# iiscleap/NeuralPlda

Hardware: AMD Instinct MI355X
Metric: scored trial-pairs/sec (512-d xvec) (higher is better)
Workload: dtype f32; 1 GPU; cfg1: 1048576 trial pairs/GPU/step, 512->150->150 NPLDA, scoring only (fused NeuralPlda.forward, inputs resident in HBM); xvector_dim=512, layer1_LDA_dim=150, layer2_PLDA_spkfactor_dim=150, params=kaldi-init truncated to 150, parallelism=trial-list shard x1, backend=single process, ranks_in_group=1

## Files before the change

neuralplda_amd/csrc/nplda_fwd_dispatch.h:

```cpp
#pragma once
#include <cstdlib>
#include "nplda_fwd_kernel.h"
#include "nplda_fwd_small.h"
#include "nplda_fwd_v2.h"
#include "nplda_fwd_v3.h"
#include "nplda_fwd_v5.h"
#include "nplda_fwd_v6.h"
#include "nplda_fwd_mid.h"

namespace nplda {

template <int MODE>
static inline int launch_fwd_v2(FwdArgs a, const NpldaLayout& L, hipStream_t st) {
    constexpr int WAVES = 8;
    const long long per_block = (MODE == MODE_EMBED ? 32 : 16) * WAVES;
    const long long blocks = (a.n + per_block - 1) / per_block;
    if (blocks > 0x7fffffffLL) return NPLDA_EINVAL;
    dim3 grid((unsigned)blocks), block(WAVES * 64);
#define NPLDA_LAUNCH(NBV) \
    hipLaunchKernelGGL((nplda_fwd_v2_kernel<NBV, MODE, WAVES, false, (NBV == 2 ? 4 : 2)>), grid, block, 0, st, a)
    switch (L.NB) {
        case 2: NPLDA_LAUNCH(2); break;
        case 4: NPLDA_LAUNCH(4); break;
        case 8: NPLDA_LAUNCH(8); break;
        case 10: NPLDA_LAUNCH(10); break;
        case 11: NPLDA_LAUNCH(11); break;
        case 12: NPLDA_LAUNCH(12); break;
        default: return NPLDA_EUNSUPPORTED;
    }
#undef NPLDA_LAUNCH
    return nplda_launch_status();
}

template <int MODE, int XM = 0>
static inline int launch_fwd_v3(FwdArgs a, const NpldaLayout& L, hipStream_t st) {
    constexpr int WAVES = 8;
    const long long per_block = (MODE == MODE_EMBED ? 32 : 16) * WAVES;
    const long long ntiles = (a.n + per_block - 1) / per_block;
    if (ntiles > 0x7fffffffLL) return NPLDA_EINVAL;
    int dev = 0, cus = 0;
    if (hipGetDevice(&dev) != hipSuccess ||
        hipDeviceGetAttribute(&cus, hipDeviceAttributeMultiprocessorCount, dev) != hipSuccess || cus <= 0)
        cus = 256;
    const long long blocks = ntiles < cus ? ntiles : cus;
    dim3 grid((unsigned)blocks), block(WAVES * 64);
#define NPLDA_LAUNCH(NBV) \
    hipLaunchKernelGGL((nplda_fwd_v3_kernel<NBV, MODE, WAVES, XM, (NBV == 2 ? 4 : 2)>), grid, block, 0, st, a, (int)ntiles)
    switch (L.NB) {
        case 2: NPLDA_LAUNCH(2); break;
        case 4: NPLDA_LAUNCH(4); break;
        case 8: NPLDA_LAUNCH(8); break;
        case 10: NPLDA_LAUNCH(10); break;
        default: return NPLDA_EUNSUPPORTED;
    }
#undef NPLDA_LAUNCH
    return nplda_launch_status();
}

template <int XM = 0>
static inline int launch_fwd_v5(FwdArgs a, const NpldaLayout& L, hipStream_t st) {
    constexpr int WAVES = 8;
    const long long ntiles = (a.n + 16 * WAVES - 1) / (16 * WAVES);
    if (ntiles > 0x7fffffffLL) return NPLDA_EINVAL;
    int dev = 0, cus = 0;
    if (hipGetDevice(&dev) != hipSuccess ||
        hipDeviceGetAttribute(&cus, hipDeviceAttributeMultiprocessorCount, dev) != hipSuccess || cus <= 0)
        cus = 256;
    const long long blocks = ntiles < cus ? ntiles : cus;
    dim3 grid((unsigned)blocks), block(WAVES * 64);
    switch (L.NB) {
        case 11: hipLaunchKernelGGL((nplda_fwd_v5_kernel<11, WAVES, 2, 6, 1, XM>), grid, block, 0, st, a, (int)ntiles); break;
        case 12: hipLaunchKernelGGL((nplda_fwd_v5_kernel<12, WAVES, 4, 4, 1, XM>), grid, block, 0, st, a, (int)ntiles); break;
        default: return NPLDA_EUNSUPPORTED;
    }
    return nplda_launch_status();
}

static inline bool fwd_v6_ok(const NpldaLayout& L) { return L.NB == 10 && L.D1 == 150 && L.D2 == 150; }
template <int XM = 0>
static inline int launch_fwd_v6(FwdArgs a, const NpldaLayout& L, hipStream_t st) {
    constexpr int WAVES = 8;
    const long long ntiles = (a.n + 16 * WAVES - 1) / (16 * WAVES);
    if (ntiles > 0x7fffffffLL) return NPLDA_EINVAL;
    if (!fwd_v6_ok(L)) return NPLDA_EUNSUPPORTED;
    int dev = 0, cus = 0;
    if (hipGetDevice(&dev) != hipSuccess ||
        hipDeviceGetAttribute(&cus, hipDeviceAttributeMultiprocessorCount, dev) != hipSuccess || cus <= 0)
        cus = 256;
    const long long blocks = ntiles < cus ? ntiles : cus;
    hipLaunchKernelGGL((nplda_fwd_v6_kernel<10, 6, WAVES, 2, 5, 3, XM>), dim3((unsigned)blocks), dim3(WAVES * 64), 0, st, a, (int)ntiles);
    return nplda_launch_status();
}
template <int XM = 0>
static inline int launch_fwd_stream(FwdArgs a, const NpldaLayout& L, hipStream_t st) {
    static const bool no_v6 = getenv("NPLDA_FWD_NO_V6") != nullptr && getenv("NPLDA_FWD_NO_V6")[0] == '1';
    if (fwd_v6_ok(L) && !no_v6) return launch_fwd_v6<XM>(a, L, st);
    if (L.NB <= 10) return launch_fwd_v3<MODE_PAIR, XM>(a, L, st);
    return launch_fwd_v5<XM>(a, L, st);
}

template <int MODE>
static inline int launch_fwd_small(FwdArgs a, const NpldaLayout& L, hipStream_t st) {
    const long long per_block = (MODE == MODE_EMBED ? 32 : 16);
    const long long blocks = (a.n + per_block - 1) / per_block;
    dim3 grid((unsigned)blocks), block(256);
#define NPLDA_LAUNCH(NBV) hipLaunchKernelGGL((nplda_fwd_small_kernel<NBV, MODE>), grid, block, 0, st, a)
#define NPLDA_LAUNCH32(NBV)                                                                           \
    if (L.KS1 == 32 && L.D0 == 512) hipLaunchKernelGGL((nplda_fwd_small_kernel<NBV, MODE, 32>), grid, block, 0, st, a); \
    else NPLDA_LAUNCH(NBV)
    switch (L.NB) {
        case 2: NPLDA_LAUNCH(2); break;
        case 4: NPLDA_LAUNCH(4); break;
        case 8: NPLDA_LAUNCH(8); break;
        case 10: NPLDA_LAUNCH32(10); break;
        case 11: NPLDA_LAUNCH32(11); break;
        case 12: NPLDA_LAUNCH(12); break;
        default: return NPLDA_EUNSUPPORTED;
    }
#undef NPLDA_LAUNCH32
#undef NPLDA_LAUNCH
    return nplda_launch_status();
}

static inline int mid_cus() {
    int dev = 0, cus = 0;
    if (hipGetDevice(&dev) != hipSuccess ||
        hipDeviceGetAttribute(&cus, hipDeviceAttributeMultiprocessorCount, dev) != hipSuccess || cus <= 0)
        cus = 256;
    return cus;
}
template <bool EMBED = false>
static inline int launch_fwd_mid(FwdArgs a, const NpldaLayout& L, hipStream_t st) {
    const long long nh = EMBED ? (a.n + 15) / 16 : (a.n + 7) / 8;
    const int cus = mid_cus();
    long long grid = nh <= cus ? nh : ((nh + 1) / 2 < cus ? (nh + 1) / 2 : cus);
    if (grid < 1) grid = 1;
    const long long c = (nh + grid - 1) / grid;
    const long long r = nh - grid * (c - 1);
    if (c > 0x7fffffffLL) return NPLDA_EINVAL;
    const bool half = !(r == grid && (c & 1) == 0);
    const bool idx = a.ia != nullptr;
#define NPLDA_LAUNCH(NBV, HV, IV) \
    hipLaunchKernelGGL((nplda_fwd_mid_kernel<NBV, EMBED, HV, IV>), dim3((unsigned)grid), dim3(256), 0, st, a, (int)c, (int)r)
#define NPLDA_LAUNCH_H(NBV, HV) do { if (idx) { NPLDA_LAUNCH(NBV, HV, true); } else { NPLDA_LAUNCH(NBV, HV, false); } } while (0)
    switch (L.NB) {
        case 10: if (half) NPLDA_LAUNCH_H(10, true); else NPLDA_LAUNCH_H(10, false); break;
        case 11: if (half) NPLDA_LAUNCH_H(11, true); else NPLDA_LAUNCH_H(11, false); break;
        default: return NPLDA_EUNSUPPORTED;
    }
#undef NPLDA_LAUNCH_H
#undef NPLDA_LAUNCH
    return nplda_launch_status();
}

template <int MODE>
static inline int launch_fwd_old(FwdArgs a, const NpldaLayout& L, hipStream_t st) {
    a.D0 = L.D0; a.KS1 = L.KS1;
    a.oW2 = L.oW2; a.ob1 = L.ob1; a.ob2 = L.ob2; a.oQ = L.oQ; a.oP = L.oP; a.total = L.total;
    const long long units = (MODE == MODE_EMBED ? (a.n + 1) / 2 : a.n);
    if (units <= 256 * 64) return launch_fwd_small<MODE>(a, L, st);
    if constexpr (MODE == MODE_PAIR) return launch_fwd_stream<0>(a, L, st);
    return launch_fwd_v2<MODE>(a, L, st);
}

enum { FWD_SMALL = 0, FWD_MID = 1, FWD_STREAM = 2, FWD_SPLIT = 3 };
static inline long long pair_split_point(long long n, int cus) { return (n / 128 / cus) * 128 * cus; }
static inline int pair_kernel_choice(long long n, const NpldaLayout& L, int cus, long long* cost = nullptr, bool allow_split = true) {
    long long dummy;
    if (!cost) cost = &dummy;
    static const bool no_mid = getenv("NPLDA_FWD_NO_MID") != nullptr && getenv("NPLDA_FWD_NO_MID")[0] == '1';
    const bool mid_ok = !no_mid && (L.NB == 10 || L.NB == 11) && L.D0 == 512 && L.KS1 == 32;
    static const long long small_max = getenv("NPLDA_FWD_SMALL_MAX") ? atoll(getenv("NPLDA_FWD_SMALL_MAX")) : -1;
    const long long round_cost = L.NB == 10 ? 1000 : 1150;
    *cost = 120;
    if (mid_ok && small_max < 0 && n <= 8LL * cus) return FWD_MID;
    *cost = 190;
    if (n <= (small_max >= 0 ? small_max : 16LL * cus)) return FWD_SMALL;
    const long long rounds = ((n + 127) / 128 + cus - 1) / cus;
    const long long t_stream = 50 + rounds * round_cost;
    *cost = n <= 64LL * cus ? 190 * ((n + 16LL * cus - 1) / (16LL * cus)) : t_stream;
    if (!mid_ok) return n <= 64LL * cus ? FWD_SMALL : FWD_STREAM;
    const long long ch = ((n + 7) / 8 + cus - 1) / cus;
    const long long t_mid = 40 + (ch / 2) * (L.NB == 10 ? 133 : 168) + (ch & 1) * (L.NB == 10 ? 93 : 118);
    int best = t_mid < t_stream ? FWD_MID : FWD_STREAM;
    *cost = t_mid < t_stream ? t_mid : t_stream;
    static const bool no_split = getenv("NPLDA_FWD_NO_SPLIT") != nullptr && getenv("NPLDA_FWD_NO_SPLIT")[0] == '1';
    const long long full = pair_split_point(n, cus);
    if (allow_split && !no_split && full > 0 && full < n) {
        long long t_rem = 0;
        pair_kernel_choice(n - full, L, cus, &t_rem, false);
        const long long t_split = 50 + (full / 128 / cus) * round_cost + t_rem;
        if (t_split + 30 < *cost) {
            *cost = t_split;
            best = FWD_SPLIT;
        }
    }
    return best;
}

template <int MODE>
static inline int launch_fwd(FwdArgs a, const NpldaLayout& L, hipStream_t st) {
    if constexpr (MODE == MODE_PAIR) {
        const int cus = mid_cus();
        const int k = pair_kernel_choice(a.n, L, cus);
        a.D0 = L.D0; a.KS1 = L.KS1;
        a.oW2 = L.oW2; a.ob1 = L.ob1; a.ob2 = L.ob2; a.oQ = L.oQ; a.oP = L.oP; a.total = L.total;
        if (k == FWD_MID) return launch_fwd_mid<false>(a, L, st);
        if (k == FWD_SMALL) return launch_fwd_small<MODE>(a, L, st);
        if (k == FWD_SPLIT && a.ia == nullptr && a.ib == nullptr) {
            const long long full = pair_split_point(a.n, cus);
            FwdArgs b = a;
            b.xa += full * a.ldx; b.xb += full * a.ldx; b.out_s += full; b.n = a.n - full;
            a.n = full;
            if (int rc = launch_fwd_stream<0>(a, L, st)) return rc;
            const int kr = pair_kernel_choice(b.n, L, cus, nullptr, false);
            if (kr == FWD_MID) return launch_fwd_mid<false>(b, L, st);
            if (kr == FWD_SMALL) return launch_fwd_small<MODE>(b, L, st);
            return launch_fwd_stream<0>(b, L, st);
        }
        return launch_fwd_stream<0>(a, L, st);
    }
    if constexpr (MODE == MODE_EMBED) {
        if (a.out_y == nullptr && pair_kernel_choice((a.n + 1) / 2, L, mid_cus(), nullptr, false) == FWD_MID) {
            a.D0 = L.D0; a.KS1 = L.KS1;
            a.oW2 = L.oW2; a.ob1 = L.ob1; a.ob2 = L.ob2; a.oQ = L.oQ; a.oP = L.oP; a.total = L.total;
            return launch_fwd_mid<true>(a, L, st);
        }
    }
    return launch_fwd_old<MODE>(a, L, st);
}

static inline int launch_fwd_pairs_bf16rows(FwdArgs a, const NpldaLayout& L, hipStream_t st) {
    const int k = pair_kernel_choice(a.n, L, mid_cus());
    if (k != FWD_STREAM && k != FWD_SPLIT) return NPLDA_EUNSUPPORTED;
    a.D0 = L.D0; a.KS1 = L.KS1;
    a.oW2 = L.oW2; a.ob1 = L.ob1; a.ob2 = L.ob2; a.oQ = L.oQ; a.oP = L.oP; a.total = L.total;
    return launch_fwd_stream<2>(a, L, st);
}

static inline const char* pair_kernel_name(long long n, const NpldaLayout& L) {
    switch (pair_kernel_choice(n, L, mid_cus())) {
        case FWD_SPLIT:
            return pair_kernel_name(pair_split_point(n, mid_cus()), L);
        case FWD_SMALL: return "nplda_fwd_small_kernel (4 waves share a 16-pair tile, feature-split)";
        case FWD_MID: return "nplda_fwd_mid_kernel (balanced 16-pair tiles, K-split layer 1, groups of 2 tiles)";
        default:
            if (fwd_v6_ok(L) && !(getenv("NPLDA_FWD_NO_V6") != nullptr && getenv("NPLDA_FWD_NO_V6")[0] == '1'))
                return "nplda_fwd_v6_kernel (persistent, 9 feature blocks on 16x16x4 MFMAs + 6 features on 4x4x1 MFMAs)";
            return L.NB <= 10 ? "nplda_fwd_v3_kernel (persistent, 8 waves x 16 pairs, weights through LDS)"
                              : "nplda_fwd_v5_kernel (persistent, LDS-DMA weight chunks, layer 2 by output groups)";
    }
}

static inline int check_model(int D0, int D1, int D2) {
    if (D0 <= 0 || D1 <= 0 || D2 <= 0 || (D0 % 4) != 0) return NPLDA_EINVAL;
    if (!nplda_dims_ok(D0, D1, D2)) return NPLDA_EUNSUPPORTED;
    return NPLDA_OK;
}

static inline bool rows_ok(const float* x, int64_t ld, int D) {
    return x && ld >= D && (ld % 4) == 0 && nplda_aligned16(x);
}

}
```

neuralplda_amd/csrc/nplda_fwd_v6.h:

```cpp
#pragma once
#include "nplda_fwd_kernel.h"

namespace nplda {

template <int NB, int TF, int WAVES, int KPB = 2, int G1 = 5, int G2 = 3, int XM = 0, int ABL = 0, int NCH = 2>
__global__ __launch_bounds__(WAVES * 64, WAVES / 4) void nplda_fwd_v6_kernel(const FwdArgs a, int ntiles) {
    constexpr int NM = NB - 1;
    constexpr int NQ = (TF + 3) / 4;
    constexpr int STEP4 = NB * 64;
    constexpr int CH1 = STEP4 * KPB;
    constexpr int NSEG1 = CH1 / 64;
    constexpr int NGR = (NM + G1 - 1) / G1;
    constexpr int NG = (NM + G2 - 1) / G2;
    constexpr int NSEG2 = NB * (G2 + 1);
    constexpr int CH2 = NSEG2 * 64;
    constexpr int CH = CH1 > CH2 ? CH1 : CH2;
    static_assert(TF >= 1 && TF <= 16 && NM >= 1 && NQ <= NGR && NQ <= NG, "tail quads ride with the MFMA groups");
    __shared__ f32x4 wbuf[2][CH];
    __shared__ f32x4 cvec[4][NB * 4];
    __shared__ f32x4 sink[64];

    const int tid = threadIdx.x;
    const int lane = tid & 63;
    const int wave = __builtin_amdgcn_readfirstlane(tid >> 6);
    const int j = lane & 15;
    const int g = lane >> 4;
    const int tl = 16 * g + (j & 3);

    const f32x4* Wall = reinterpret_cast<const f32x4*>(a.packed);
    const long long w2base4 = (long long)(a.oW2 / 4);
    for (int i = tid; i < 4 * NB * 4; i += WAVES * 64) {
        const int v = i / (NB * 4), e = i % (NB * 4);
        const size_t o = v == 0 ? a.ob1 : (v == 1 ? a.ob2 : (v == 2 ? a.oQ : a.oP));
        cvec[v][e] = reinterpret_cast<const f32x4*>(a.packed + o)[e];
    }
    const f32x4* b1p = cvec[0];
    const f32x4* b2p = cvec[1];
    const f32x4* Qp = cvec[2];
    const f32x4* Pp = cvec[3];
    const int KS1 = a.KS1;
    const int D0 = a.D0;
    const int NC1 = (KS1 + KPB - 1) / KPB;

    auto seg_dma = [&](const f32x4* src, f32x4* dst) {
        unsigned lo = (unsigned)lane * 16u;
        asm volatile("" : "+v"(lo));
        __builtin_amdgcn_global_load_lds((const __attribute__((address_space(1))) void*)(reinterpret_cast<const char*>(src) + lo),
                                         (__attribute__((address_space(3))) void*)dst, 16, 0, 0);
    };
    auto dma_l1 = [&](int c, f32x4* dst) {
        const f32x4* src = Wall + (long long)c * CH1;
#pragma unroll
        for (int i = 0; i < (NSEG1 + WAVES - 1) / WAVES; ++i) {
            const int sgm = wave + WAVES * i;
            const bool live = sgm < NSEG1;
            seg_dma(src + (live ? sgm : 0) * 64, live ? dst + sgm * 64 : sink);
        }
    };
    auto dma_l2 = [&](int nb0, int gc, f32x4* dst) {
        const int per = gc + 1;
        const int nseg = NB * per;
#pragma unroll
        for (int i = 0; i < (NSEG2 + WAVES - 1) / WAVES; ++i) {
            const int sgm = wave + WAVES * i;
            const bool live = sgm < nseg;
            const int sg = live ? sgm : 0;
            const int kb = sg / per, u = sg - kb * per;
            const int blk = u < gc ? nb0 + u : NM;
            seg_dma(Wall + w2base4 + (long long)kb * STEP4 + blk * 64, live ? dst + sgm * 64 : sink);
        }
    };
    auto chunk_fence = [&]() {
        __builtin_amdgcn_s_waitcnt(0x0070);
        __builtin_amdgcn_s_barrier();
        __builtin_amdgcn_sched_barrier(0);
    };
    auto kgroups_sum = [&](float v) {
        v = wave_xor_add(v, 16);
        return wave_xor_add(v, 32);
    };
    auto as_block = [&](const float (&u)[TF]) {
        f32x4 blk = {0.f, 0.f, 0.f, 0.f};
#pragma unroll
        for (int r = 0; r < 4; ++r) {
#pragma unroll
            for (int gg = 0; gg < 4; ++gg)
                if (4 * gg + r < TF) blk[r] = (g == gg) ? u[4 * gg + r] : blk[r];
        }
        return blk;
    };

    auto tile_rows = [&](long long t, long long& t0, long long& r) {
        t0 = (t * WAVES + wave) * 16;
        r = t0 + j;
    };
    long long tile = blockIdx.x;
    long long t0, row;
    tile_rows(tile, t0, row);
    bool ok = row < a.n;
    if (!ok) row = a.n - 1;
    const float* sa = x_row<XM>(a.xa, row, a.ldx);
    const float* sb = x_row<XM>(a.xb, row, a.ldx);

    dma_l1(0, wbuf[0]);
    f32x4 xa[KPB], xb[KPB];
#pragma unroll
    for (int s = 0; s < KPB; ++s) {
        xa[s] = load_xrow<XM>(sa, 16 * s + 4 * g, D0);
        xb[s] = load_xrow<XM>(sb, 16 * s + 4 * g, D0);
    }
    __syncthreads();
    chunk_fence();
    int par = 0;

    for (;;) {
        const long long tile_n = tile + gridDim.x;
        long long t0_n, row_n;
        tile_rows(tile_n, t0_n, row_n);
        const bool ok_n = row_n < a.n;
        if (!ok_n) row_n = a.n - 1;
        const float* sa_n = x_row<XM>(a.xa, row_n, a.ldx);
        const float* sb_n = x_row<XM>(a.xb, row_n, a.ldx);

        f32x4 accA[NB], accB[NB];
#pragma unroll
        for (int nb = 0; nb < NM; ++nb) {
            accA[nb] = b1p[4 * nb + g];
            accB[nb] = accA[nb];
        }
        f32x4 qA[NQ][NCH], qB[NQ][NCH];
#pragma unroll
        for (int q = 0; q < NQ; ++q) {
#pragma unroll
            for (int h = 0; h < NCH; ++h) {
                qA[q][h] = f32x4{0.f, 0.f, 0.f, 0.f};
                qB[q][h] = qA[q][h];
            }
        }

        auto chunk = [&](int c, f32x4 (&xc)[KPB], f32x4 (&yc)[KPB], f32x4 (&xn)[KPB], f32x4 (&yn)[KPB]) {
            const bool more = (c + 1 < NC1);
            f32x4* nxt = wbuf[par ^ 1];
            if (more) dma_l1(c + 1, nxt);
            else dma_l2(0, (G2 < NM ? G2 : NM), nxt);
#pragma unroll
            for (int s = 0; s < KPB; ++s) {
                const int ks = more ? KPB * (c + 1) + s : KPB * c + s;
                xn[s] = load_xrow<XM>(sa, 16 * ks + 4 * g, D0);
                yn[s] = load_xrow<XM>(sb, 16 * ks + 4 * g, D0);
            }
            const f32x4* w = wbuf[par];
#pragma unroll
            for (int s = 0; s < KPB; ++s) {
                if (KPB * c + s < KS1) {
#pragma unroll
                    for (int gr = 0; gr < NGR; ++gr) {
                        const int nb0 = gr * G1;
                        f32x4 av[G1];
#pragma unroll
                        for (int u = 0; u < G1; ++u)
                            if (nb0 + u < NM) av[u] = w[s * STEP4 + (nb0 + u) * 64 + lane];
#pragma unroll
                        for (int r = 0; r < 4; ++r) {
#pragma unroll
                            for (int u = 0; u < G1; ++u) {
                                if (nb0 + u < NM) {
                                    accA[nb0 + u] = __builtin_amdgcn_mfma_f32_16x16x4f32(av[u][r], xc[s][r], accA[nb0 + u], 0, 0, 0);
                                    accB[nb0 + u] = __builtin_amdgcn_mfma_f32_16x16x4f32(av[u][r], yc[s][r], accB[nb0 + u], 0, 0, 0);
                                }
                            }
                        }
                        if (gr < NQ && ABL != 1) {
                            const f32x4 wq = w[s * STEP4 + NM * 64 + tl + 4 * gr];
#pragma unroll
                            for (int r = 0; r < 4; ++r) {
                                qA[gr][r % NCH] = __builtin_amdgcn_mfma_f32_4x4x1f32(wq[r], xc[s][r], qA[gr][r % NCH], 0, 0, 0);
                                qB[gr][r % NCH] = __builtin_amdgcn_mfma_f32_4x4x1f32(wq[r], yc[s][r], qB[gr][r % NCH], 0, 0, 0);
                            }
                        }
                    }
                }
            }
            chunk_fence();
            par ^= 1;
        };
        f32x4 xan[KPB], xbn[KPB];
        int c = 0;
        for (; c + 1 < NC1; c += 2) {
            chunk(c, xa, xb, xan, xbn);
            chunk(c + 1, xan, xbn, xa, xb);
        }
        if (c < NC1) {
            chunk(c, xa, xb, xan, xbn);
#pragma unroll
            for (int s = 0; s < KPB; ++s) {
                xa[s] = xan[s];
                xb[s] = xbn[s];
            }
        }

        {
            float uA[TF], uB[TF];
#pragma unroll
            for (int f = 0; f < TF; ++f) {
                float sa_ = qA[f / 4][0][f % 4], sb_ = qB[f / 4][0][f % 4];
#pragma unroll
                for (int h = 1; h < NCH; ++h) {
                    sa_ += qA[f / 4][h][f % 4];
                    sb_ += qB[f / 4][h][f % 4];
                }
                uA[f] = kgroups_sum(sa_);
                uB[f] = kgroups_sum(sb_);
            }
            const f32x4 bt = b1p[4 * NM + g];
            accA[NM] = as_block(uA) + bt;
            accB[NM] = as_block(uB) + bt;
        }

        {
            float ssA = 0.f, ssB = 0.f;
#pragma unroll
            for (int nb = 0; nb < NB; ++nb) {
#pragma unroll
                for (int r = 0; r < 4; ++r) {
                    ssA = fmaf(accA[nb][r], accA[nb][r], ssA);
                    ssB = fmaf(accB[nb][r], accB[nb][r], ssB);
                }
            }
            ssA = wave_xor_add(ssA, 16); ssA = wave_xor_add(ssA, 32);
            ssB = wave_xor_add(ssB, 16); ssB = wave_xor_add(ssB, 32);
            const float invA = 1.0f / fmaxf(sqrtf(ssA), 1e-12f);
            const float invB = 1.0f / fmaxf(sqrtf(ssB), 1e-12f);
#pragma unroll
            for (int nb = 0; nb < NB; ++nb) {
                accA[nb] *= invA;
                accB[nb] *= invB;
            }
        }

        float part = 0.f;
#pragma unroll
        for (int gi = 0; gi < NG; ++gi) {
            const int nb0 = gi * G2;
            const int gc = (NM - nb0) < G2 ? (NM - nb0) : G2;
            const int per = gc + 1;
            f32x4 zA[G2], zB[G2];
#pragma unroll
            for (int u = 0; u < G2; ++u) {
                if (u < gc) {
                    zA[u] = b2p[4 * (nb0 + u) + g];
                    zB[u] = zA[u];
                }
            }
            f32x4 zqA[2] = {{0.f, 0.f, 0.f, 0.f}, {0.f, 0.f, 0.f, 0.f}}, zqB[2] = {{0.f, 0.f, 0.f, 0.f}, {0.f, 0.f, 0.f, 0.f}};
            f32x4* nxt = wbuf[par ^ 1];
            if (gi + 1 < NG) {
                const int nb1 = nb0 + G2;
                dma_l2(nb1, (NM - nb1) < G2 ? (NM - nb1) : G2, nxt);
            } else {
                dma_l1(0, nxt);
#pragma unroll
                for (int s = 0; s < KPB; ++s) {
                    xa[s] = load_xrow<XM>(sa_n, 16 * s + 4 * g, D0);
                    xb[s] = load_xrow<XM>(sb_n, 16 * s + 4 * g, D0);
                }
            }
            const f32x4* w = wbuf[par];
#pragma unroll
            for (int kb = 0; kb < NB; ++kb) {
                f32x4 av[G2];
#pragma unroll
                for (int u = 0; u < G2; ++u)
                    if (u < gc) av[u] = w[(kb * per + u) * 64 + lane];
#pragma unroll
                for (int r = 0; r < 4; ++r) {
#pragma unroll
                    for (int u = 0; u < G2; ++u) {
                        if (u < gc) {
                            zA[u] = __builtin_amdgcn_mfma_f32_16x16x4f32(av[u][r], accA[kb][r], zA[u], 0, 0, 0);
                            zB[u] = __builtin_amdgcn_mfma_f32_16x16x4f32(av[u][r], accB[kb][r], zB[u], 0, 0, 0);
                        }
                    }
                }
                if (gi < NQ && ABL != 1) {
                    const f32x4 wq = w[(kb * per + gc) * 64 + tl + 4 * gi];
#pragma unroll
                    for (int r = 0; r < 4; ++r) {
                        zqA[r & 1] = __builtin_amdgcn_mfma_f32_4x4x1f32(wq[r], accA[kb][r], zqA[r & 1], 0, 0, 0);
                        zqB[r & 1] = __builtin_amdgcn_mfma_f32_4x4x1f32(wq[r], accB[kb][r], zqB[r & 1], 0, 0, 0);
                    }
                }
            }
            chunk_fence();
            par ^= 1;
#pragma unroll
            for (int u = 0; u < G2; ++u) {
                if (u < gc) {
                    const f32x4 q = Qp[4 * (nb0 + u) + g];
                    const f32x4 p = Pp[4 * (nb0 + u) + g];
#pragma unroll
                    for (int r = 0; r < 4; ++r) {
                        const float z1 = zA[u][r], z2 = zB[u][r];
                        part = fmaf(q[r], fmaf(z1, z1, z2 * z2), part);
                        part = fmaf(2.0f * p[r], z1 * z2, part);
                    }
                }
            }
            if (gi < NQ) {
                float tpart = 0.f;
                const float* b2s = reinterpret_cast<const float*>(b2p);
                const float* Qs = reinterpret_cast<const float*>(Qp);
                const float* Ps = reinterpret_cast<const float*>(Pp);
#pragma unroll
                for (int i = 0; i < 4; ++i) {
                    const int f = 4 * gi + i;
                    if (f < TF) {
                        const float z1 = kgroups_sum(zqA[0][i] + zqA[1][i]) + b2s[16 * NM + f];
                        const float z2 = kgroups_sum(zqB[0][i] + zqB[1][i]) + b2s[16 * NM + f];
                        tpart = fmaf(Qs[16 * NM + f], fmaf(z1, z1, z2 * z2), tpart);
                        tpart = fmaf(2.0f * Ps[16 * NM + f], z1 * z2, tpart);
                    }
                }
                part += (g == 0) ? tpart : 0.f;
            }
        }
        part = wave_xor_add(part, 16);
        part = wave_xor_add(part, 32);
        if (g == 0 && ok) a.out_s[t0 + j] = part;

        tile = tile_n;
        if (tile >= ntiles) break;
        t0 = t0_n; ok = ok_n;
        sa = sa_n; sb = sb_n;
    }
}

}
```

Measured before the change: 335.2 million pairs/s.

## Run NPLDA layer 2 as split-bf16x3 MFMAs with W2 staged through LDS

Adds an L2S path to the v6 persistent kernel, enabled by default, that computes layer 2 with bf16x3 split-precision 16x16x32 MFMAs (6 passes) instead of the f32 grouped path. W2 chunks are loaded from global memory per wave, split into hi/mid/lo bf16 in registers and double-buffered in LDS. The next tile's layer-1 weight DMA and x-row loads are overlapped with the layer-2 loop. The aim is to cut the f32 MFMA cost of layer 2 while keeping roughly f32 accuracy through the three-way split, at the cost of extra split arithmetic and more LDS. The old f32 path stays reachable via an environment variable.

```diff
diff --git a/neuralplda_amd/csrc/nplda_fwd_dispatch.h b/neuralplda_amd/csrc/nplda_fwd_dispatch.h
--- a/neuralplda_amd/csrc/nplda_fwd_dispatch.h
+++ b/neuralplda_amd/csrc/nplda_fwd_dispatch.h
@@ -1,5 +1,6 @@
 #pragma once
 #include <cstdlib>
+#include <cstring>
 #include "nplda_fwd_kernel.h"
 #include "nplda_fwd_small.h"
 #include "nplda_fwd_v2.h"
@@ -77,6 +78,10 @@
 }
 
 static inline bool fwd_v6_ok(const NpldaLayout& L) { return L.NB == 10 && L.D1 == 150 && L.D2 == 150; }
+static inline bool fwd_v6_l2_f32() {
+    static const bool f32 = getenv("NPLDA_FWD_V6_L2") != nullptr && strcmp(getenv("NPLDA_FWD_V6_L2"), "f32") == 0;
+    return f32;
+}
 template <int XM = 0>
 static inline int launch_fwd_v6(FwdArgs a, const NpldaLayout& L, hipStream_t st) {
     constexpr int WAVES = 8;
@@ -88,7 +93,12 @@
         hipDeviceGetAttribute(&cus, hipDeviceAttributeMultiprocessorCount, dev) != hipSuccess || cus <= 0)
         cus = 256;
     const long long blocks = ntiles < cus ? ntiles : cus;
-    hipLaunchKernelGGL((nplda_fwd_v6_kernel<10, 6, WAVES, 2, 5, 3, XM>), dim3((unsigned)blocks), dim3(WAVES * 64), 0, st, a, (int)ntiles);
+    if (fwd_v6_l2_f32())
+        hipLaunchKernelGGL((nplda_fwd_v6_kernel<10, 6, WAVES, 2, 5, 3, XM, 0, 2, 0>), dim3((unsigned)blocks), dim3(WAVES * 64), 0, st, a,
+                           (int)ntiles);
+    else
+        hipLaunchKernelGGL((nplda_fwd_v6_kernel<10, 6, WAVES, 2, 5, 3, XM, 0, 2, 1>), dim3((unsigned)blocks), dim3(WAVES * 64), 0, st, a,
+                           (int)ntiles);
     return nplda_launch_status();
 }
 template <int XM = 0>
@@ -246,7 +256,10 @@
         case FWD_MID: return "nplda_fwd_mid_kernel (balanced 16-pair tiles, K-split layer 1, groups of 2 tiles)";
         default:
             if (fwd_v6_ok(L) && !(getenv("NPLDA_FWD_NO_V6") != nullptr && getenv("NPLDA_FWD_NO_V6")[0] == '1'))
-                return "nplda_fwd_v6_kernel (persistent, 9 feature blocks on 16x16x4 MFMAs + 6 features on 4x4x1 MFMAs)";
+                return fwd_v6_l2_f32()
+                           ? "nplda_fwd_v6_kernel (persistent, 9 feature blocks on 16x16x4 MFMAs + 6 features on 4x4x1 MFMAs)"
+                           : "nplda_fwd_v6_kernel (persistent, layer 1: 9 feature blocks on 16x16x4 MFMAs + 6 features on 4x4x1 "
+                             "MFMAs; layer 2: split bf16x3, 6 passes of 16x16x32)";
             return L.NB <= 10 ? "nplda_fwd_v3_kernel (persistent, 8 waves x 16 pairs, weights through LDS)"
                               : "nplda_fwd_v5_kernel (persistent, LDS-DMA weight chunks, layer 2 by output groups)";
     }
diff --git a/neuralplda_amd/csrc/nplda_fwd_v6.h b/neuralplda_amd/csrc/nplda_fwd_v6.h
--- a/neuralplda_amd/csrc/nplda_fwd_v6.h
+++ b/neuralplda_amd/csrc/nplda_fwd_v6.h
@@ -1,9 +1,11 @@
 #pragma once
 #include "nplda_fwd_kernel.h"
+#include "nplda_fwd_bf16x3.h"
 
 namespace nplda {
 
-template <int NB, int TF, int WAVES, int KPB = 2, int G1 = 5, int G2 = 3, int XM = 0, int ABL = 0, int NCH = 2>
+template <int NB, int TF, int WAVES, int KPB = 2, int G1 = 5, int G2 = 3, int XM = 0, int ABL = 0, int NCH = 2,
+          int L2S = 0>
 __global__ __launch_bounds__(WAVES * 64, WAVES / 4) void nplda_fwd_v6_kernel(const FwdArgs a, int ntiles) {
     constexpr int NM = NB - 1;
     constexpr int NQ = (TF + 3) / 4;
@@ -13,10 +15,14 @@
     constexpr int NGR = (NM + G1 - 1) / G1;
     constexpr int NG = (NM + G2 - 1) / G2;
     constexpr int NSEG2 = NB * (G2 + 1);
-    constexpr int CH2 = NSEG2 * 64;
+    constexpr int CH2 = L2S ? 0 : NSEG2 * 64;
     constexpr int CH = CH1 > CH2 ? CH1 : CH2;
+    constexpr int KC2 = NB / 2;
     static_assert(TF >= 1 && TF <= 16 && NM >= 1 && NQ <= NGR && NQ <= NG, "tail quads ride with the MFMA groups");
+    static_assert(!L2S || (NB % 2 == 0 && WAVES <= NB && NB <= 2 * WAVES), "split layer 2: k32-steps of two whole accumulator "
+                                                                            "blocks, one or two W2 units per wave");
     __shared__ f32x4 wbuf[2][CH];
+    __shared__ bf16x8 wsp[L2S ? 2 : 1][L2S ? NB * 3 * 64 : 1];
     __shared__ f32x4 cvec[4][NB * 4];
     __shared__ f32x4 sink[64];
 
@@ -75,6 +81,24 @@
         __builtin_amdgcn_s_barrier();
         __builtin_amdgcn_sched_barrier(0);
     };
+    f32x4 w2lo[2], w2hi[2];
+    const bool two = wave + WAVES < NB;
+    auto w2_load = [&](int c, int i, int r) {
+        const int nb = wave + WAVES * i;
+        const char* base = reinterpret_cast<const char*>(Wall + w2base4 + (long long)(2 * c) * STEP4 + (nb < NB ? nb : 0) * 64);
+        unsigned lo = (unsigned)lane * 16u;
+        asm volatile("" : "+v"(lo));
+        w2lo[r] = *reinterpret_cast<const f32x4*>(base + lo);
+        w2hi[r] = *reinterpret_cast<const f32x4*>(base + STEP4 * 16 + lo);
+    };
+    auto w2_store = [&](int i, int r, bf16x8* dst) {
+        const int nb = wave + WAVES * i;
+        bf16x8 h, m, l;
+        split3x8(w2lo[r], w2hi[r], h, m, l);
+        dst[(nb * 3 + 0) * 64 + lane] = h;
+        dst[(nb * 3 + 1) * 64 + lane] = m;
+        dst[(nb * 3 + 2) * 64 + lane] = l;
+    };
     auto kgroups_sum = [&](float v) {
         v = wave_xor_add(v, 16);
         return wave_xor_add(v, 32);
@@ -94,13 +118,19 @@
         t0 = (t * WAVES + wave) * 16;
         r = t0 + j;
     };
+    auto tile_ptrs = [&](long long t, long long& t0, bool& ok, const float*& pa, const float*& pb) {
+        long long r;
+        tile_rows(t, t0, r);
+        ok = r < a.n;
+        if (!ok) r = a.n - 1;
+        pa = x_row<XM>(a.xa, r, a.ldx);
+        pb = x_row<XM>(a.xb, r, a.ldx);
+    };
     long long tile = blockIdx.x;
-    long long t0, row;
-    tile_rows(tile, t0, row);
-    bool ok = row < a.n;
-    if (!ok) row = a.n - 1;
-    const float* sa = x_row<XM>(a.xa, row, a.ldx);
-    const float* sb = x_row<XM>(a.xb, row, a.ldx);
+    long long t0;
+    bool ok;
+    const float *sa, *sb;
+    tile_ptrs(tile, t0, ok, sa, sb);
 
     dma_l1(0, wbuf[0]);
     f32x4 xa[KPB], xb[KPB];
@@ -115,12 +145,10 @@
 
     for (;;) {
         const long long tile_n = tile + gridDim.x;
-        long long t0_n, row_n;
-        tile_rows(tile_n, t0_n, row_n);
-        const bool ok_n = row_n < a.n;
-        if (!ok_n) row_n = a.n - 1;
-        const float* sa_n = x_row<XM>(a.xa, row_n, a.ldx);
-        const float* sb_n = x_row<XM>(a.xb, row_n, a.ldx);
+        long long t0_n;
+        bool ok_n;
+        const float *sa_n, *sb_n;
+        tile_ptrs(tile_n, t0_n, ok_n, sa_n, sb_n);
 
         f32x4 accA[NB], accB[NB];
 #pragma unroll
@@ -142,6 +170,10 @@
             const bool more = (c + 1 < NC1);
             f32x4* nxt = wbuf[par ^ 1];
             if (more) dma_l1(c + 1, nxt);
+            else if constexpr (L2S) {
+                w2_load(0, 0, 0);
+                w2_load(0, 1, 1);
+            }
             else dma_l2(0, (G2 < NM ? G2 : NM), nxt);
 #pragma unroll
             for (int s = 0; s < KPB; ++s) {
@@ -181,6 +213,12 @@
                     }
                 }
             }
+            if constexpr (L2S) {
+                if (!more) {
+                    w2_store(0, 0, wsp[0]);
+                    if (two) w2_store(1, 1, wsp[0]);
+                }
+            }
             chunk_fence();
             par ^= 1;
         };
@@ -239,6 +277,64 @@
         }
 
         float part = 0.f;
+        if constexpr (L2S) {
+            f32x4 zA[NB], zB[NB];
+#pragma unroll
+            for (int nb = 0; nb < NB; ++nb) {
+                zA[nb] = b2p[4 * nb + g];
+                zB[nb] = zA[nb];
+            }
+#pragma unroll
+            for (int c = 0; c < KC2; ++c) {
+                const bool more = c + 1 < KC2;
+                if (more) {
+                    w2_load(c + 1, 0, 0);
+                } else {
+                    dma_l1(0, wbuf[par]);
+                    long long t0_x;
+                    bool ok_x;
+                    const float *pa, *pb;
+                    tile_ptrs(tile_n, t0_x, ok_x, pa, pb);
+#pragma unroll
+                    for (int s = 0; s < KPB; ++s) {
+                        xa[s] = load_xrow<XM>(pa, 16 * s + 4 * g, D0);
+                        xb[s] = load_xrow<XM>(pb, 16 * s + 4 * g, D0);
+                    }
+                }
+                bf16x8 ah, am, al, bh, bm, bl;
+                split3x8(accA[2 * c], accA[2 * c + 1], ah, am, al);
+                split3x8(accB[2 * c], accB[2 * c + 1], bh, bm, bl);
+                const bf16x8* w = wsp[c & 1];
+#pragma unroll
+                for (int nb = 0; nb < NB; nb += 2) {
+                    WFrag w0, w1;
+                    w0.h = w[(nb * 3 + 0) * 64 + lane];
+                    w0.m = w[(nb * 3 + 1) * 64 + lane];
+                    w0.l = w[(nb * 3 + 2) * 64 + lane];
+                    w1.h = w[(nb * 3 + 3) * 64 + lane];
+                    w1.m = w[(nb * 3 + 4) * 64 + lane];
+                    w1.l = w[(nb * 3 + 5) * 64 + lane];
+                    mfma6x4(w0, w1, ah, am, al, bh, bm, bl, zA[nb], zB[nb], zA[nb + 1], zB[nb + 1]);
+                    if (more && nb == 2 * ((NB / 2) / 2)) {
+                        w2_store(0, 0, wsp[(c + 1) & 1]);
+                        w2_load(c + 1, 1, 0);
+                    }
+                }
+                if (more && two) w2_store(1, 0, wsp[(c + 1) & 1]);
+                chunk_fence();
+            }
+#pragma unroll
+            for (int nb = 0; nb < NB; ++nb) {
+                const f32x4 q = Qp[4 * nb + g];
+                const f32x4 p = Pp[4 * nb + g];
+#pragma unroll
+                for (int r = 0; r < 4; ++r) {
+                    const float z1 = zA[nb][r], z2 = zB[nb][r];
+                    part = fmaf(q[r], fmaf(z1, z1, z2 * z2), part);
+                    part = fmaf(2.0f * p[r], z1 * z2, part);
+                }
+            }
+        } else {
 #pragma unroll
         for (int gi = 0; gi < NG; ++gi) {
             const int nb0 = gi * G2;
@@ -324,14 +420,19 @@
                 part += (g == 0) ? tpart : 0.f;
             }
         }
+        }
         part = wave_xor_add(part, 16);
         part = wave_xor_add(part, 32);
         if (g == 0 && ok) a.out_s[t0 + j] = part;
 
         tile = tile_n;
         if (tile >= ntiles) break;
-        t0 = t0_n; ok = ok_n;
-        sa = sa_n; sb = sb_n;
+        if constexpr (L2S) {
+            tile_ptrs(tile, t0, ok, sa, sb);
+        } else {
+            t0 = t0_n; ok = ok_n;
+            sa = sa_n; sb = sb_n;
+        }
     }
 }
 
```

Result: faster. 362.6 million pairs/s, median of 6 (+8.2%).
